# NathanBWaters/playaid_core

Measured on AMD Instinct MI355X. Metric: 1080p frames/sec end-to-end, higher is better.
Workload: dtype f32; 1 GPU; configs[1]: 64 x 1080x1920 BGR frames per GPU per clip; parallelism=single GPU, lanes=2, ingest=raw BGR frames resident in HBM

## Files before the change

### playaid_core_amd/csrc/engine_plan.h

```cpp
#pragma once
#include "gemm_tile.h"

#include <algorithm>
#include <cstddef>
#include <cstdlib>

namespace pa {

constexpr int WINO_F4_MIN_CROPS = 64;

struct EngineKnobs {
    int patch = 1;
    int bf16_patch = 1;
    int bf16_t256 = 1;
    int s2_pgemm = 2;
    int stem_igemm = 0;
    int stem_pool = 1;
    int pool_overlap = 1;
    int ds_side = 0;
    int stem_int = 1;
    int wino = 1;
    int wino_min_hw = 4;
    int wino_ds = 1;
    int wino_f4 = 1;
    int wino_f4_min = WINO_F4_MIN_CROPS;
    int bf16_ds_fuse = 1;
    int f32_ds_fuse = 1;
    bool profile_layers = false;
    int force_tile = -1;
    int force_splitk = 0;
    int fc_splitk = 0;
    int head_splitk = 0;
    int interleave = 0;
};

inline int env_int(const char* name, int unset) {
    const char* v = getenv(name);
    return v ? atoi(v) : unset;
}
inline int env_min1(const char* name) {
    const char* v = getenv(name);
    return v ? std::max(1, atoi(v)) : 0;
}

inline EngineKnobs engine_knobs() {
    static const EngineKnobs once = [] {
        EngineKnobs k;
        k.patch = env_int("PA_PATCH", k.patch);
        k.bf16_patch = env_int("PA_BF16_PATCH", k.bf16_patch);
        k.bf16_t256 = env_int("PA_BF16_T256", k.bf16_t256);
        k.s2_pgemm = env_int("PA_S2_PGEMM", k.s2_pgemm);
        k.stem_igemm = env_int("PA_STEM_IGEMM", k.stem_igemm);
        k.stem_pool = env_int("PA_STEM_POOL", k.stem_pool);
        k.pool_overlap = env_int("PA_POOL_OVERLAP", k.pool_overlap);
        k.ds_side = env_int("PA_DS_SIDE", k.ds_side);
        k.stem_int = env_int("PA_STEM_INT", k.stem_int);
        k.wino = env_int("PA_WINO", k.wino);
        k.wino_min_hw = env_int("PA_WINO_MIN_HW", k.wino_min_hw);
        k.wino_ds = env_int("PA_WINO_DS", k.wino_ds);
        k.wino_f4 = env_int("PA_WINO_F4", k.wino_f4);
        k.wino_f4_min = env_int("PA_WINO_F4_MIN", k.wino_f4_min);
        k.bf16_ds_fuse = env_int("PA_BF16_DS_FUSE", k.bf16_ds_fuse);
        k.f32_ds_fuse = env_int("PA_F32_DS_FUSE", k.f32_ds_fuse);
        return k;
    }();
    EngineKnobs k = once;
    const char* pl = getenv("PA_PROFILE_LAYERS");
    k.profile_layers = pl && pl[0] == '1';
    k.force_tile = env_int("PA_FORCE_TILE", -1);
    k.force_splitk = env_min1("PA_FORCE_SPLITK");
    k.fc_splitk = env_min1("PA_FC_SPLITK");
    k.head_splitk = env_min1("PA_HEAD_SPLITK");
    k.interleave = env_int("PA_INTERLEAVE", 0);
    return k;
}

enum ComputeDtype { DT_F32, DT_EMULATED_F32, DT_BF16 };

struct EngineForms {
    bool stem_fused;
    bool stem_int;
    bool opener_branch;
};
inline EngineForms engine_forms(const EngineKnobs& k, ComputeDtype dt) {
    EngineForms f;
    f.stem_fused = k.stem_pool && !k.stem_igemm;
    f.stem_int = dt != DT_BF16 && k.stem_int && f.stem_fused;
    f.opener_branch = dt == DT_BF16 ? k.bf16_ds_fuse != 0 : dt == DT_F32 && k.f32_ds_fuse && !k.ds_side && k.s2_pgemm;
    return f;
}

enum BranchPlace {
    BRANCH_NONE,
    BRANCH_SECOND_K,
// ... 209 lines not shown
```

### playaid_core_amd/csrc/pa_api.hip

```cpp
#include "../../include/playaid_hip.h"
#include "conv_rows.h"
#include "engine_table.h"
#include "synth_math.h"
#include "train_common.h"

#include <algorithm>
#include <cmath>
#include <cstdio>
#include <cstdlib>
#include <cstring>
#include <string>
#include <vector>

using namespace pa;

namespace {

static_assert(FEATURE_STRIDE == PA_FEATURE_STRIDE, "engine_table.h pads the fc to the cached feature rows' width");
constexpr int WINO_TICKETS = 4096;

struct ConvLayer : LayerDesc {
    std::string name;
    float* in = nullptr;
    float* out = nullptr;
// ... 246 lines not shown
            on = false;
            return;
        }
        (void)hipEventRecord(ent.start, s);
    }
    ~ProfScope() {
        if (!on) return;
        (void)hipEventRecord(ent.stop, s);
        e->prof_log.push_back(ent);
    }
};

float* buf_at(float* base, size_t elems, bool bf) { return reinterpret_cast<float*>(reinterpret_cast<char*>(base) + elems * (bf ? 2 : 4)); }

bool branch_on_side(const pa_engine* e, hipStream_t s) { return e->knobs.ds_side && !e->profiling && !e->bf16 && e->side && s != e->side; }

int run_branch_gemm(pa_engine* e, const ConvLayer& L, const BranchPlan& b, int crop0, int ncrops, size_t slab_off, hipStream_t s, const char* prof_name) {
    const int hw = L.branch.hw, c = L.branch.c, out_w = L.out_hw + 2 * L.out_pad;
    const size_t out_crop = (size_t)out_w * out_w * L.cout;
    GemmParams d = conv_row_params({ ncrops,  hw, hw, 1, c,
                                     c, L.cout, 1, L.branch.stride,
                                     L.out_pad, L.cout,  0, 0});
    d.act = buf_at(L.ds.src, (size_t)crop0 * (hw + 2) * (hw + 2) * c, e->bf16);
    d.wgt = L.ds.wgt;
    d.out = buf_at(L.ds.out, crop0 * out_crop, e->bf16);
    d.slab = e->slab + slab_off;
    ProfScope ps(e, s, prof_name, b.acct.flops, b.acct.bytes);
    if (e->bf16) HIPCHK(e, launch_igemm_bf16(d, b.tile, s));
    else if (b.psgemm) HIPCHK(e, launch_psgemm(d, L.ds.split_wgt, (size_t)ncrops * out_crop, 0, s));
    else HIPCHK(e, launch_igemm(d, b.tile, s));
    return PA_OK;
}

int run_conv(pa_engine* e, const ConvLayer& L, int crop0, int ncrops, size_t slab_off, hipStream_t s, const char* prof_name) {
    const size_t slab_avail = e->slab_floats > slab_off ? e->slab_floats - slab_off : 0;
    const ConvPlan P = plan_conv(e->knobs, e->dtype, L, ncrops, slab_avail, branch_on_side(e, s));
    const bool bf = e->bf16 && L.kh == 3;
    const int in_w = L.in_hw + 2 * L.in_pad;
    const int out_w = L.out_hw + 2 * L.out_pad;
    const size_t in_crop = (size_t)in_w * in_w * L.in_px_stride;
    const size_t out_crop = (size_t)out_w * out_w * L.cout;
    GemmParams p;
    memset(&p, 0, sizeof(p));
    p.act = buf_at(L.in, crop0 * in_crop, bf);
    p.wgt = L.wgt;
    p.bias = L.bias;
    p.residual = L.residual ? buf_at(L.residual, crop0 * out_crop, bf) : nullptr;
    p.out = buf_at(L.out, crop0 * out_crop, bf);
    p.slab = e->slab + slab_off;
    p.gather = nullptr;
    p.M = P.M;
    p.N = P.N;
    p.taps = L.taps;
    p.kw_taps = L.kw_taps;
    p.chunk = L.chunk;
    p.ktot = P.ktot;
    p.skip_w = L.kh == 7;
    p.howo = L.out_hw * L.out_hw;
    p.wo = L.out_hw;
    p.in_px_stride = L.in_px_stride;
    p.in_row_stride = in_w * L.in_px_stride;
    p.in_img_stride = (int)in_crop;
    p.stride = L.stride;
    p.off_y = L.off;
    p.off_x = L.off;
    p.out_px_stride = L.cout;
    p.out_row_stride = out_w * L.cout;
// ... 7 lines not shown
    }
    if (P.branch == BL_GEMM_BEFORE || P.branch == BL_STORED) {
        p.residual = buf_at(L.ds.out, crop0 * out_crop, bf);
    } else if (P.branch == BL_SECOND_K) {
        const int w2 = L.branch.hw + 2;
        p.act2 = buf_at(L.ds.src, (size_t)crop0 * w2 * w2 * L.branch.c, bf);
        p.k2_steps = L.branch.c / (bf ? 64 : 32);
        p.in2_px_stride = L.branch.c;
        p.in2_row_stride = w2 * L.branch.c;
        p.in2_img_stride = w2 * w2 * L.branch.c;
        p.stride2 = L.branch.stride;
        p.off2 = 1;
    }
    const ConvLayer* C2 = L.carries_of >= 0 ? &e->convs[L.carries_of] : nullptr;
    if (bf && P.branch == BL_ON_OPENER) {
        p.wgt2 = C2->ds.wgt;
        p.out2 = buf_at(C2->ds.out, crop0 * out_crop, bf);
    }
    bool branch_left = P.branch == BL_GEMM_BEHIND;
    {
        ProfScope ps(e, s, prof_name, P.acct.flops, P.acct.bytes, P.acct.flops_executed);
        hipError_t pe = hipErrorInvalidValue;
        if (P.form == CONV_PSGEMM) {
            pe = launch_psgemm(p, L.split_wgt, (size_t)ncrops * out_crop, 0, s);
        } else if (P.form == CONV_WINO && P.wino_f4) {
            Wino4Params q{};
            q.act = p.act; q.wgt = L.wino4_wgt; q.bias = p.bias; q.residual = p.residual; q.out = p.out;
            q.v = e->wino4_scratch + (slab_off ? e->wino4_region : 0);
            q.m = q.v + (size_t)36 * wino4_rows(ncrops) * L.cin;
            q.n_img = ncrops; q.cin = L.cin; q.cout = L.cout;
            q.in_px_stride = p.in_px_stride; q.in_row_stride = p.in_row_stride; q.in_img_stride = p.in_img_stride;
            q.out_px_stride = p.out_px_stride; q.out_row_stride = p.out_row_stride; q.out_img_stride = p.out_img_stride; q.out_pad = p.out_pad;
            q.relu = p.relu; q.res_after = p.res_after;
            pe = launch_wino4_conv3x3(q, s);
        } else if (P.form == CONV_WINO) {
            WinoParams q = wino_params(p, ncrops, L.out_hw, L.out_hw, L.cin, L.wino_wgt, L.wino_bn);
            if (e->wino_tickets && e->slab) {
                q.slab = e->slab + slab_off;
                q.slab_floats = e->slab_floats > slab_off ? std::min(e->slab_floats - slab_off, e->slab_floats / 2) : 0;
                q.tickets = reinterpret_cast<int32_t*>(e->wino_tickets) + (slab_off ? WINO_TICKETS : 0);
                q.tickets_cap = WINO_TICKETS;
            }
            pe = launch_wino3x3(q, s);
        } else if (bf) {
            if (P.form == CONV_BF16_PATCH) pe = launch_conv3x3_bf16_patch(p, s);
            if (pe == hipErrorInvalidValue) pe = launch_igemm_bf16(p, P.tile_256 ? TILE_256x128 : P.tile, s);
        } else {
            if (P.form == CONV_PATCH) pe = launch_conv3x3_patch(p, P.patch_bm, s);
            if (P.form == CONV_PGEMM && P.branch == BL_ON_OPENER) {
                p.wgt2 = C2->ds.wgt;
                p.out2 = buf_at(C2->ds.out, crop0 * out_crop, bf);
                pe = launch_pgemm(p, 64, s);
                branch_left = pe != hipSuccess;
                p.wgt2 = nullptr;
                p.out2 = nullptr;
            }
            if (P.form == CONV_PGEMM && pe == hipErrorInvalidValue) pe = launch_pgemm(p, P.pgemm_bm, s);
            if (pe == hipErrorInvalidValue) pe = launch_igemm(p, P.tile, s);
        }
        HIPCHK(e, pe);
    }
    if (branch_left) return run_branch_gemm(e, *C2, P.branch_gemm, crop0, ncrops, slab_off, s, e->knobs.profile_layers ? C2->name.c_str() : prof_name);
    return PA_OK;
}

int run_backbone_part(pa_engine* e, int crop0, int ncrops, const float* x_in, float* feats_out, size_t slab_off, hipStream_t s,
// ... 32 lines not shown
        memset(&sp, 0, sizeof(sp));
        const size_t es_in = x_form ? 2 : 4, es_out = e->bf16 ? 2 : 4;
        sp.x = reinterpret_cast<const char*>(x_in) + (size_t)crop0 * 134 * 134 * 4 * es_in;
        sp.wgt = x_form == 2 ? (const void*)e->stem_wgt_int : e->bf16 ? (const void*)e->stem_wgt_bf16 : (const void*)stem.wgt;
        sp.bias = stem.bias;
        sp.out = reinterpret_cast<char*>(e->p1) + (size_t)crop0 * 34 * 34 * 64 * es_out;
        sp.crops = ncrops;
        sp.in_bf16 = x_form;
        sp.out_bf16 = e->bf16 ? 1 : 0;
        const double px = (double)ncrops * 64 * 64;
        ProfScope ps(e, s, "stem_conv7x7_pool", 2.0 * px * 64 * 147,
                     (double)es_in * ((double)ncrops * 128 * 128 * 4 + 64.0 * 147 * (x_form == 2 ? 3 : 1)) + (double)es_out * ncrops * 32 * 32 * 64);
        HIPCHK(e, launch_stem_pool(sp, s));
    } else if (x_form == 2) {
        return fail(e, PA_ERR_INVALID_ARG, "integer pixels reached an unfused stem (PA_STEM_POOL=0 / PA_STEM_IGEMM=1 switch the integer stem off)");
    } else if (e->bf16) {
        return fail(e, PA_ERR_INVALID_ARG, "the bf16 path has no unfused stem (PA_STEM_POOL=0 / PA_STEM_IGEMM=1 are fp32 A/B knobs)");
    } else if (K.pool_overlap && !e->profiling && !K.interleave && e->side && s != e->side && ncrops >= 64) {
        const int half = (ncrops / 2 + 7) & ~7;
        if ((rc = stem_part(crop0, half, s))) return rc;
        HIPCHK(e, hipEventRecord(e->ev_fork, s));
        HIPCHK(e, hipStreamWaitEvent(e->side, e->ev_fork, 0));
        if ((rc = pool_part(crop0, half, e->side))) return rc;
        HIPCHK(e, hipEventRecord(e->ev_join, e->side));
        if ((rc = stem_part(crop0 + half, ncrops - half, s))) return rc;
        if ((rc = pool_part(crop0 + half, ncrops - half, s))) return rc;
        HIPCHK(e, hipStreamWaitEvent(s, e->ev_join, 0));
    } else {
        if ((rc = stem_part(crop0, ncrops, s))) return rc;
        if ((rc = pool_part(crop0, ncrops, s))) return rc;
    }
    if (stop <= 1) return PA_OK;
    const bool on_side = branch_on_side(e, s);
    for (size_t i = 1; i < e->convs.size(); ++i) {
        const ConvLayer& L = e->convs[i];
        const char* pn = K.profile_layers ? L.name.c_str() : (L.kh == 3 ? "igemm_conv3x3" : "igemm_conv1x1_ds");
        const bool side_next = on_side && i + 1 < e->convs.size() && e->convs[i + 1].branch.place == BRANCH_OWN_GEMM;
        if (side_next) {
            const ConvLayer& Nx = e->convs[i + 1];
            HIPCHK(e, hipEventRecord(e->ev_ds_fork, s));
            HIPCHK(e, hipStreamWaitEvent(e->side, e->ev_ds_fork, 0));
            if ((rc = run_branch_gemm(e, Nx, plan_branch(e->dtype, Nx, ncrops), crop0, ncrops, slab_off, e->side, "igemm_conv1x1_ds"))) return rc;
            HIPCHK(e, hipEventRecord(e->ev_ds_join, e->side));
        }
        if (on_side && L.branch.place == BRANCH_OWN_GEMM) HIPCHK(e, hipStreamWaitEvent(s, e->ev_ds_join, 0));
        if ((rc = run_conv(e, L, crop0, ncrops, slab_off, s, pn))) return rc;
        if (stop <= (int)i + 1) {
            if (side_next) HIPCHK(e, hipStreamWaitEvent(s, e->ev_ds_join, 0));
            return PA_OK;
        }
    }
    {
        ProfScope ps(e, s, "avgpool", 0.0, ncrops * ((e->bf16 ? 2.0 : 4.0) * 16.0 * 512 + 4.0 * 512));
        if (e->bf16)
            HIPCHK(e, launch_avgpool_bf16(reinterpret_cast<uint16_t*>(e->layer4_out) + (size_t)crop0 * 36 * 512,
                                          e->pooled + (size_t)crop0 * 512, ncrops, s));
        else
            HIPCHK(e, launch_avgpool(e->layer4_out + (size_t)crop0 * 36 * 512, e->pooled + (size_t)crop0 * 512, ncrops, s));
    }
    if (stop <= 18) return PA_OK;
    ConvLayer fc = e->fc;
    fc.out = feats_out;
    rc = run_conv(e, fc, crop0, ncrops, slab_off, s, "igemm_fc");
    return rc;
}

int run_backbone(pa_engine* e, int ncrops, const float* x_in, float* feats_out, hipStream_t s, int stop = PA_TRACE_STAGES) {
    if (!e->knobs.interleave || ncrops < 64 || !e->side) return run_backbone_part(e, 0, ncrops, x_in, feats_out, 0, s, stop);
    const int half = (ncrops / 2 + 7) & ~7;
    HIPCHK(e, hipEventRecord(e->ev_fork, s));
    HIPCHK(e, hipStreamWaitEvent(e->side, e->ev_fork, 0));
    int rc = run_backbone_part(e, 0, half, x_in, feats_out, 0, s, stop);
    if (rc) return rc;
    rc = run_backbone_part(e, half, ncrops - half, x_in, feats_out, e->slab_floats / 2, e->side, stop);
    if (rc) return rc;
    HIPCHK(e, hipEventRecord(e->ev_join, e->side));
    HIPCHK(e, hipStreamWaitEvent(s, e->ev_join, 0));
    return PA_OK;
}
// ... 1649 lines not shown
```

### playaid_core_amd/csrc/pa_kernels.h

```cpp
#pragma once
#include "gemm_tile.h"
#include <hip/hip_runtime.h>
#include <stdint.h>
#include "crop_math.h"

namespace pa {

__device__ __forceinline__ float silu_fast(float x) {
    return x * __builtin_amdgcn_rcpf(1.0f + __builtin_amdgcn_exp2f(x * -1.44269504088896341f));
}

struct GemmParams {
    const float* act;
    const float* wgt;
    const float* bias;
    const float* residual;
    float* out;
    float* slab;
    const int32_t* gather;
    int32_t M, N, ktot;
    int32_t taps, kw_taps, chunk;
    int32_t howo, wo;
    int32_t howo_shift, wo_shift;
    int32_t in_img_stride, in_row_stride, in_px_stride, stride, off_y, off_x;
// ... 82 lines not shown
    float* out;
    int32_t n_img, height, width, cin, cout;
    int32_t bn;
    int32_t in_px_stride, in_row_stride, in_img_stride;
    int32_t out_px_stride, out_row_stride, out_img_stride, out_pad;
    int32_t relu, res_after;
    int32_t n_sb, sb_per_row, sb_per_img, tiles_n;
    unsigned long long* clk;
    float* slab;
    size_t slab_floats;
    int32_t* tickets;
    int32_t tickets_cap, ksplit;
    int32_t tiles_m, xcd_gm, xcd_gn;
};
size_t wino_weight_floats(int cin, int cout);
int wino_pick_bn(int cout, long long n_sb, int cin_split = 0);
void wino_transform_weights(const float* w, int cin, int cout, int bn, float* ug);
hipError_t launch_wino3x3(const WinoParams& p, hipStream_t s);

struct Wino4Params {
    const float* act;
    const float* wgt;
    const float* bias;
    const float* residual;
    float* out;
    float* v;
    float* m;
    int32_t n_img, cin, cout;
    int32_t in_px_stride, in_row_stride, in_img_stride;
    int32_t out_px_stride, out_row_stride, out_img_stride, out_pad;
    int32_t relu, res_after;
    int32_t tile;
    int32_t rows;
};
size_t wino4_weight_floats(int cin, int cout);
int wino4_rows(int n_img);
void wino4_transform_weights(const float* w, int cin, int cout, float* u);
hipError_t launch_wino4_conv3x3(const Wino4Params& p, hipStream_t s);

#define PA_FUSED_LDS_BYTES 77824

#define PA_HOP_BLOCKS_MAX 48
#define PA_HOP_PIXELS 10
#define PA_HOP_WINDOW 64
#define PA_HOP_BLOCK_BYTES (6 * 1024 + 32 * 4 + 16)
#define PA_CROP_MFMA_H_DEFAULT 1

struct CropWindow {
    int64_t offset;
    int32_t pitch;
    int32_t rows;
    int64_t src_offset;
    int32_t src_pitch;
    int32_t row_bytes;
};
hipError_t launch_slice_upload(const uint8_t* frames_host, long long frames_bytes, const CropWindow* desc, uint8_t* windows, int ncrops,
                               hipStream_t s);

struct PreprocParams {
    const uint8_t* frames;
    const CropWindow* windows;
    const double* boxes;
    const int32_t* src_frame;
    int32_t n_src;
    int32_t n_frames, height, width, fighters, padding, swap_rb;
    CropPlan* plans;
// ... 229 lines not shown
```

### playaid_core_amd/csrc/pigemm.hip

```cpp
#include "pgemm_common.h"

#include <algorithm>
#include <type_traits>
#include <cstdio>
#include <cstdlib>
#include <vector>

namespace pa {


namespace {

typedef __attribute__((address_space(3))) float lds_f32;
typedef __attribute__((address_space(3))) f32x4 lds_f32x4;

template <int N> __device__ __forceinline__ void pg_wait_vm() { wait_vmcnt<(N > 63 ? 63 : N)>(); }

}

template <int BM, int BN, bool SILU, bool STAMP, bool UP, bool DS, bool GRP = false>
__device__ __forceinline__ void pgemm_body(const GemmParams& p) {
    static_assert(!DS || (!UP && !STAMP && !SILU), "the branch form is the ResNet openers': ReLU, no up-sampled copy");
    static_assert(!GRP || (!UP && !STAMP && !SILU && !DS), "the grouped form is a plain product");
    auto stamp = [&](int i) {
        if (STAMP) {
            const unsigned long long t = __builtin_amdgcn_s_memtime();
            if ((threadIdx.x & 63) == 0) p.clk[((size_t)blockIdx.x * 4 + (threadIdx.x >> 6)) * 64 + i] = t;
        }
    };
    stamp(0);
    constexpr int WM = BN == 64 ? 2 : 4;
    constexpr int MI = BM / WM / 32;
    constexpr int A_ROWS = BM / 32, B_ROWS = BN / 32;
    constexpr int NLD = A_ROWS + B_ROWS;
    constexpr int NST = MI * 4 * (UP ? 5 : (DS ? 2 : 1));
    constexpr int STAGE = (BM + BN + (DS ? BN : 0)) * 32;
    __shared__ __attribute__((aligned(16))) float lds[3 * STAGE];

    const TileRun run = tile_run(p);
    const int tile_n = run.tile_n, nt = run.nt;
    {
        const float *pa_ = p.act, *pw_ = p.wgt, *pb_ = p.bias;
        float* po_ = p.out;
        const int i0 = p.M, i1 = p.ktot, i2 = p.kw_taps, i3 = p.chunk, i4 = p.howo, i5 = p.wo, i6 = p.in_img_stride, i7 = p.in_row_stride,
                  i8 = p.in_px_stride, i9 = p.stride, i10 = p.off_y, i11 = p.off_x, i12 = p.out_img_stride, i13 = p.out_row_stride,
                  i14 = p.out_px_stride, i15 = p.out_pad, i16 = p.pg_ho, i17 = p.pg_nwx, i18 = p.pg_nwy;
        const unsigned u0 = p.pg_magic_howo, u1 = p.pg_magic_wo;
        asm volatile("" ::"s"(pa_), "s"(pw_), "s"(pb_), "s"(po_), "s"(i0), "s"(i1), "s"(i2), "s"(i3), "s"(i4), "s"(i5), "s"(i6), "s"(i7), "s"(i8), "s"(i9),
                     "s"(i10), "s"(i11), "s"(i12), "s"(i13), "s"(i14), "s"(i15), "s"(i16), "s"(i17), "s"(i18), "s"(u0), "s"(u1));
        if (DS) {
            const float* pw2_ = p.wgt2;
            float* po2_ = p.out2;
            asm volatile("" ::"s"(pw2_), "s"(po2_));
        }
        if (GRP) {
            const int g0 = p.grp_tiles, g1 = p.grp_wgt_bytes;
// ... 73 lines not shown
        const int tapoff = cur.tap_offset(p) * 4;
#pragma unroll
        for (int i = 0; i < A_ROWS; ++i) glds16(act_rs, a_off[i], tapoff, As_w + i * 1024);
        const int koff = ((cur.ky * p.kw_taps + cur.kx) * p.chunk + cur.kc) * 4 + (GRP ? w_grp : 0);
#pragma unroll
        for (int i = 0; i < B_ROWS; ++i) glds16(wgt_rs, b_off[i], koff, Bs_w + i * 1024);
        if (DS && cur.ky == 1 && cur.kx == 1) {
#pragma unroll
            for (int i = 0; i < B_ROWS; ++i) glds16(wgt2_rs, b2_off[i], cur.kc * 4, Bs_w + BN * 32 + i * 1024);
        }
        cur.advance(p, nk, run, rows_of);
    };

    unsigned a_k[4], b_k[4];
    {
        const int a_rd = (wm * (BM / WM) + lr) * 32, b_rd = BM * 32 + (wn * 32 + lr) * 32;
        const int swz = (lr >> 1) & 7;
        const unsigned base = (unsigned)(size_t)(lds_f32*)lds;
#pragma unroll
        for (int kk = 0; kk < 4; ++kk) {
            const int ch_ = ((kk * 2 + lh) ^ swz) * 4;
            a_k[kk] = base + (a_rd + ch_) * 4;
            b_k[kk] = base + (b_rd + ch_) * 4;
            asm volatile("" : "+v"(a_k[kk]), "+v"(b_k[kk]));
        }
    }

    issue(0);
    stamp(62);
    if (total > 1) issue(1);
    f32x16 biasv;
#pragma unroll
    for (int g = 0; g < 4; ++g) {
        const f32x4 b4 = p.bias ? *reinterpret_cast<const f32x4*>(p.bias + ch0 + 8 * g) : f32x4{0.f, 0.f, 0.f, 0.f};
        biasv[4 * g] = b4.x; biasv[4 * g + 1] = b4.y; biasv[4 * g + 2] = b4.z; biasv[4 * g + 3] = b4.w;
    }
    asm volatile("" : "+v"(biasv));
    stamp(1);

    f32x16 acc[MI];
    f32x16 acc2[MI];
    f32x16 accg[GRP ? 3 : 1][MI];
    auto kstep = [&](int sb, auto first_c, auto branch_c) {
        constexpr bool FIRST = decltype(first_c)::value;
        constexpr int BR = decltype(branch_c)::value;
        f32x16 zero16;
        if (BR == 1) {
#pragma unroll
            for (int e = 0; e < 16; ++e) zero16[e] = 0.f;
        }
        f32x4 b2f[2];
        unsigned ra[4], rb[4];
#pragma unroll
        for (int kk = 0; kk < 4; ++kk) {
            ra[kk] = a_k[kk] + sb;
            rb[kk] = b_k[kk] + sb;
            asm volatile("" : "+v"(ra[kk]), "+v"(rb[kk]));
        }
        f32x4 af[2][MI], bf[2];
#define PG_FRAGS(SET, KK)                                                                                    \
    {                                                                                                        \
        _Pragma("unroll") for (int mi = 0; mi < MI; ++mi)                                                    \
            af[SET][mi] = *(const lds_f32x4*)(size_t)(ra[KK] + mi * 4096);                                   \
        bf[SET] = *(const lds_f32x4*)(size_t)(rb[KK]);                                                       \
        if (BR) b2f[SET] = *(const lds_f32x4*)(size_t)(rb[KK] + BN * 128);                                    \
    }
        PG_FRAGS(0, 0);
#pragma unroll
        for (int kk = 0; kk < 4; ++kk) {
#pragma unroll
// ... 83 lines not shown
            }
            if (DS && live) {
                float* o2_px = p.out2 + o_off;
#pragma unroll
                for (int gq = 0; gq < 4; ++gq)
                    *reinterpret_cast<f32x4*>(o2_px + 8 * gq) = f32x4{acc2[mi][4 * gq], acc2[mi][4 * gq + 1], acc2[mi][4 * gq + 2], acc2[mi][4 * gq + 3]};
            }
            if (UP && live) {
                float* u_px = p.up_out + pixel_walk(geom, m_base, lr, p.up_img_stride, up_rs, up_ps, up_wrap_x, up_wrap_y, up_lane);
#pragma unroll
                for (int q4 = 0; q4 < 4; ++q4) {
                    float* u = u_px + (q4 >> 1) * p.up_row_stride + (q4 & 1) * p.up_px_stride;
#pragma unroll
                    for (int gq = 0; gq < 4; ++gq) *reinterpret_cast<f32x4*>(u + 8 * gq) = out4[gq];
                }
            }
        }
        if (t < 15) stamp(5 + 4 * t);
    }
    stamp(63);
}

template <int BM, int BN = 64, bool SILU = true, bool STAMP = false, bool UP = false>
__global__ __launch_bounds__(256, 2) void pgemm_kernel(const GemmParams p) {
    pgemm_body<BM, BN, SILU, STAMP, UP, false>(p);
}

__global__ __launch_bounds__(256, 2) void pgemm_branch_kernel(const GemmParams p) {
    pgemm_body<64, 64, false, false, false, true>(p);
}

template <int BM, int BN>
__global__ __launch_bounds__(256, 2) void pgemm_group_kernel(const GemmParams p) {
    pgemm_body<BM, BN, false, false, false, false, true>(p);
}

hipError_t launch_pgemm(const GemmParams& p_in, int bm, hipStream_t s) {
    GemmParams p = p_in;
    if (p.residual || p.N % 32 != 0 || (bm != 128 && bm != 64 && bm != 0) || persistent_plan(p) != hipSuccess) return hipErrorInvalidValue;
    const bool branch = p.wgt2 || p.out2;
    if (branch) {
        if (!p.wgt2 || !p.out2 || p.taps != 9 || p.kw_taps != 3 || p.stride != 2 || p.in_px_stride != p.chunk || p.splitk > 1 || p.N % 64 != 0 || p.relu == 2 || p.up_out ||
            ((reinterpret_cast<unsigned long long>(p.wgt2) | reinterpret_cast<unsigned long long>(p.out2)) & 15ull))
            return hipErrorInvalidValue;
        bm = 64;
    }
    const int bn = p.N % 64 == 0 ? 64 : 32;
    if (bn == 32) bm = 128;
    p.tiles_n = p.N / bn;
    if (p.tiles_n > 64) return hipErrorInvalidValue;
    auto plan = [&](int bm_, int* lm_out) {
        const int tm = (p.M + bm_ - 1) / bm_, share = (tm + 7) / 8;
        int lm = 64 / p.tiles_n;
        lm = lm < 1 ? 1 : (lm > share ? share : lm);
        *lm_out = lm;
        return (double)((share + lm - 1) / lm) * (bm_ == 128 ? 1.0 : 0.55) * (lm * p.tiles_n <= 32 ? 0.6 : 1.0);
    };
    int lm = 1;
    if (bm == 0) {
        int lm128, lm64;
        const double e128 = plan(128, &lm128), e64 = plan(64, &lm64);
        bm = e128 <= e64 ? 128 : 64;
        lm = bm == 128 ? lm128 : lm64;
    } else {
        (void)plan(bm, &lm);
    }
    p.tiles_m = (p.M + bm - 1) / bm;
// ... 45 lines not shown
hipError_t launch_pgemm_grouped(const float* a, const float* w, float* out, int groups, int rows, int K, int N, int tile, hipStream_t s) {
    auto mis = [](const void* q) { return (reinterpret_cast<unsigned long long>(q) & 15ull) != 0; };
    if (!a || !w || !out || mis(a) || mis(w) || mis(out) || groups < 1 || rows < 64 || rows % 64 || rows >= (1 << 16) || K < 32 || K % 32 || N < 64 || N % 64 ||
        tile < 0 || tile > 3)
        return hipErrorInvalidValue;
    if ((long long)groups * rows * K * 4 >= (1ll << 31) || (long long)groups * N * K * 4 >= (1ll << 31) || (long long)groups * rows * N >= (1ll << 31))
        return hipErrorInvalidValue;
    if (tile == 0) tile = 1;
    if (tile != 1 && rows % 128) tile = 1;
    const int bm = tile == 1 ? 64 : 128, bn = tile == 3 ? 32 : 64;
    GemmParams p;
    memset(&p, 0, sizeof(p));
    p.act = a; p.wgt = w; p.out = out;
    p.M = groups * rows; p.N = N; p.ktot = K;
    p.taps = 1; p.kw_taps = 1; p.chunk = K;
    p.howo = rows; p.wo = rows;
    p.in_px_stride = K; p.in_row_stride = rows * K; p.in_img_stride = rows * K; p.stride = 1;
    p.out_px_stride = N; p.out_row_stride = rows * N; p.out_img_stride = rows * N;
    p.splitk = 1;
    if (persistent_plan(p) != hipSuccess) return hipErrorInvalidValue;
    p.tiles_n = N / bn;
    p.tiles_m = p.M / bm;
    if (p.tiles_n > 64) return hipErrorInvalidValue;
    p.grp_tiles = rows / bm;
    p.grp_wgt_bytes = N * K * 4;
    p.grp_magic = (unsigned)std::min<unsigned long long>(((1ull << 32) + p.grp_tiles - 1) / p.grp_tiles, 0xffffffffull);
    const int share = (p.tiles_m + 7) / 8;
    int lm = 96 / p.tiles_n;
    static const int lm_force = getenv("PA_PGEMM_GROUP_LM") ? atoi(getenv("PA_PGEMM_GROUP_LM")) : 0;
    if (lm_force > 0) lm = lm_force;
    lm = lm < 1 ? 1 : (lm > share ? share : lm);
    p.pg_per = lm * p.tiles_n;
    const int grid = p.pg_per * 8;
    if (tile == 1) hipLaunchKernelGGL((pgemm_group_kernel<64, 64>), dim3(grid), dim3(256), 0, s, p);
    else if (tile == 2) hipLaunchKernelGGL((pgemm_group_kernel<128, 64>), dim3(grid), dim3(256), 0, s, p);
    else hipLaunchKernelGGL((pgemm_group_kernel<128, 32>), dim3(grid), dim3(256), 0, s, p);
    return hipGetLastError();
}

}
```

### playaid_core_amd/csrc/wino4.hip

```cpp
#include "tile_common.h"

#include <cstdlib>

namespace pa {

namespace {

__device__ __forceinline__ f32x4 w4_fma(float a, f32x4 x, f32x4 y) {
    return f32x4{__builtin_fmaf(a, x.x, y.x), __builtin_fmaf(a, x.y, y.y), __builtin_fmaf(a, x.z, y.z), __builtin_fmaf(a, x.w, y.w)};
}

__device__ __forceinline__ void w4_bt(f32x4 (&d)[6]) {
    const f32x4 t0 = w4_fma(4.f, d[0], w4_fma(-5.f, d[2], d[4]));
    const f32x4 t5 = w4_fma(4.f, d[1], w4_fma(-5.f, d[3], d[5]));
    const f32x4 a = w4_fma(-4.f, d[2], d[4]), b = w4_fma(-4.f, d[1], d[3]);
    const f32x4 c = d[4] - d[2], e = d[3] - d[1];
    d[0] = t0; d[1] = a + b; d[2] = a - b; d[3] = w4_fma(2.f, e, c); d[4] = w4_fma(-2.f, e, c); d[5] = t5;
}

__device__ __forceinline__ void w4_at(const f32x4 (&m)[6], f32x4 (&y)[4]) {
    const f32x4 s = m[1] + m[2], d = m[1] - m[2], u = m[3] + m[4], v = m[3] - m[4];
    y[0] = (m[0] + s) + u;
    y[1] = w4_fma(2.f, v, d);
    y[2] = w4_fma(4.f, u, s);
    y[3] = w4_fma(8.f, v, d) + m[5];
}

__global__ __launch_bounds__(64) void wino4_input_kernel(const Wino4Params p) {
    const int cq_n = p.cin >> 2;
    const int idx = blockIdx.x * 64 + threadIdx.x;
    const int row = idx / cq_n, c = (idx - row * cq_n) * 4;
    if (row >= p.rows) return;
    float* v = p.v + (size_t)row * p.cin + c;
    const size_t plane = (size_t)p.rows * p.cin;
    if (row >= p.n_img) {
#pragma unroll
        for (int q = 0; q < 36; ++q) *reinterpret_cast<f32x4*>(v + q * plane) = f32x4{0.f, 0.f, 0.f, 0.f};
        return;
    }
    const float* x = p.act + (size_t)row * p.in_img_stride + c;
    f32x4 d[6][6];
#pragma unroll
    for (int i = 0; i < 6; ++i)
#pragma unroll
        for (int j = 0; j < 6; ++j) d[i][j] = *reinterpret_cast<const f32x4*>(x + i * p.in_row_stride + j * p.in_px_stride);
#pragma unroll
    for (int j = 0; j < 6; ++j) {
        f32x4 l[6];
#pragma unroll
        for (int i = 0; i < 6; ++i) l[i] = d[i][j];
        w4_bt(l);
#pragma unroll
        for (int i = 0; i < 6; ++i) d[i][j] = l[i];
    }
#pragma unroll
    for (int i = 0; i < 6; ++i) {
        w4_bt(d[i]);
#pragma unroll
        for (int j = 0; j < 6; ++j) *reinterpret_cast<f32x4*>(v + (i * 6 + j) * plane) = d[i][j];
    }
}

__global__ __launch_bounds__(64) void wino4_output_kernel(const Wino4Params p) {
    const int cq_n = p.cout >> 2;
    const int idx = blockIdx.x * 64 + threadIdx.x;
    const int row = idx / cq_n, c = (idx - row * cq_n) * 4;
    if (row >= p.n_img) return;
    const float* m = p.m + (size_t)row * p.cout + c;
    const size_t plane = (size_t)p.rows * p.cout;
    f32x4 t[4][6];
#pragma unroll
    for (int j = 0; j < 6; ++j) {
        f32x4 l[6], y[4];
#pragma unroll
        for (int i = 0; i < 6; ++i) l[i] = *reinterpret_cast<const f32x4*>(m + (i * 6 + j) * plane);
        w4_at(l, y);
#pragma unroll
        for (int i = 0; i < 4; ++i) t[i][j] = y[i];
    }
    const f32x4 bias4 = p.bias ? *reinterpret_cast<const f32x4*>(p.bias + c) : f32x4{0.f, 0.f, 0.f, 0.f};
    const size_t o00 = (size_t)row * p.out_img_stride + (size_t)p.out_pad * (p.out_row_stride + p.out_px_stride) + c;
    f32x4 res4[4][4];
#pragma unroll
    for (int oy = 0; oy < 4; ++oy)
#pragma unroll
        for (int ox = 0; ox < 4; ++ox)
            res4[oy][ox] = p.residual ? *reinterpret_cast<const f32x4*>(p.residual + o00 + (size_t)oy * p.out_row_stride + ox * p.out_px_stride)
                                      : f32x4{0.f, 0.f, 0.f, 0.f};
#pragma unroll
    for (int oy = 0; oy < 4; ++oy) {
        f32x4 y[4];
        w4_at(t[oy], y);
#pragma unroll
        for (int ox = 0; ox < 4; ++ox)
            *reinterpret_cast<f32x4*>(p.out + o00 + (size_t)oy * p.out_row_stride + ox * p.out_px_stride) = epilogue4(y[ox], bias4, res4[oy][ox], p.relu, p.res_after);
    }
}

}

size_t wino4_weight_floats(int cin, int cout) { return (size_t)36 * cin * cout; }

int wino4_rows(int n_img) { return (n_img + 63) / 64 * 64; }

void wino4_transform_weights(const float* w, int cin, int cout, float* u) {
    static const double Gm[6][3] = {{1.0 / 4, 0, 0},          {-1.0 / 6, -1.0 / 6, -1.0 / 6}, {-1.0 / 6, 1.0 / 6, -1.0 / 6},
                                    {1.0 / 24, 1.0 / 12, 1.0 / 6}, {1.0 / 24, -1.0 / 12, 1.0 / 6},  {0, 0, 1}};
    const size_t plane = (size_t)cout * cin;
    for (int co = 0; co < cout; ++co)
        for (int ci = 0; ci < cin; ++ci) {
            double g[3][3], tmp[6][3];
            for (int ky = 0; ky < 3; ++ky)
                for (int kx = 0; kx < 3; ++kx) g[ky][kx] = (double)w[((size_t)co * 9 + ky * 3 + kx) * cin + ci];
            for (int i = 0; i < 6; ++i)
                for (int kx = 0; kx < 3; ++kx) tmp[i][kx] = Gm[i][0] * g[0][kx] + Gm[i][1] * g[1][kx] + Gm[i][2] * g[2][kx];
            for (int i = 0; i < 6; ++i)
                for (int j = 0; j < 6; ++j)
                    u[(size_t)(i * 6 + j) * plane + (size_t)co * cin + ci] = (float)(tmp[i][0] * Gm[j][0] + tmp[i][1] * Gm[j][1] + tmp[i][2] * Gm[j][2]);
        }
}

hipError_t launch_wino4_conv3x3(const Wino4Params& p_in, hipStream_t s) {
    Wino4Params p = p_in;
    if (!p.act || !p.wgt || !p.out || !p.v || !p.m || p.n_img < 1 || p.cin < 64 || p.cin % 64 || p.cout < 64 || p.cout % 64 || p.in_px_stride < p.cin ||
        p.out_px_stride < p.cout || p.out_pad < 0)
        return hipErrorInvalidValue;
    auto mis = [](const void* q) { return (reinterpret_cast<unsigned long long>(q) & 15ull) != 0; };
    if (p.in_px_stride % 4 || p.out_px_stride % 4 || p.in_row_stride % 4 || p.in_img_stride % 4 || p.out_row_stride % 4 || p.out_img_stride % 4 || mis(p.act) ||
        mis(p.wgt) || mis(p.out) || mis(p.v) || mis(p.m) || (p.bias && mis(p.bias)) || (p.residual && mis(p.residual)))
        return hipErrorInvalidValue;
    p.rows = wino4_rows(p.n_img);
    const long long in_threads = (long long)p.rows * (p.cin / 4), out_threads = (long long)p.n_img * (p.cout / 4);
    if (in_threads >= (1ll << 31) || out_threads >= (1ll << 31)) return hipErrorInvalidValue;
    hipLaunchKernelGGL(wino4_input_kernel, dim3((unsigned)((in_threads + 63) / 64)), dim3(64), 0, s, p);
    static const int tile_env = getenv("PA_WINO_F4_TILE") ? atoi(getenv("PA_WINO_F4_TILE")) : 0;
    const hipError_t e = launch_pgemm_grouped(p.v, p.wgt, p.m, 36, p.rows, p.cin, p.cout, p.tile ? p.tile : tile_env, s);
    if (e != hipSuccess) return e;
    hipLaunchKernelGGL(wino4_output_kernel, dim3((unsigned)((out_threads + 63) / 64)), dim3(64), 0, s, p);
    return hipGetLastError();
}

}

#include "../../include/playaid_hip.h"

extern "C" {

size_t pa_wino4_weight_floats(int32_t cin, int32_t cout) {
    if (cin < 64 || cin % 64 || cout < 64 || cout % 64) return 0;
    return pa::wino4_weight_floats(cin, cout);
}

int pa_wino4_transform_weights(const float* w_host, int32_t cin, int32_t cout, float* u_host) {
    if (!w_host || !u_host || cin < 64 || cin % 64 || cout < 64 || cout % 64) return PA_ERR_INVALID_ARG;
    pa::wino4_transform_weights(w_host, cin, cout, u_host);
    return PA_OK;
}

int pa_wino4_conv3x3(const float* x, const float* u, const float* bias, const float* residual, float* out, int32_t n, int32_t height, int32_t width,
                     int32_t cin, int32_t cout, int32_t in_px_stride, int32_t out_px_stride, int32_t out_pad, int32_t act, int32_t res_after,
                     float* scratch, size_t scratch_floats, void* stream) {
    if (!x || !u || !out || !scratch || n < 1 || height != 4 || width != 4 || out_pad < 0 || act < 0 || act > 2 || cin < 64 || cin % 64 || cout < 64 ||
        cout % 64 || (reinterpret_cast<unsigned long long>(scratch) & 15ull))
        return PA_ERR_INVALID_ARG;
    const size_t rows = (size_t)pa::wino4_rows(n);
    if (scratch_floats < 36 * rows * ((size_t)cin + cout)) return PA_ERR_INVALID_ARG;
    pa::Wino4Params p{};
    p.act = x; p.wgt = u; p.bias = bias; p.residual = residual; p.out = out;
    p.v = scratch;
    p.m = scratch + 36 * rows * cin;
    p.n_img = n; p.cin = cin; p.cout = cout;
// ... 15 lines not shown
```

Baseline: 75100 frames/s.

## Chain Winograd F4 layers by fusing next input transform into output kernel

New measurement: 74810 frames/s. Within noise of the previous version (-0.4%).

```diff
diff --git a/playaid_core_amd/csrc/engine_plan.h b/playaid_core_amd/csrc/engine_plan.h
--- a/playaid_core_amd/csrc/engine_plan.h
+++ b/playaid_core_amd/csrc/engine_plan.h
@@ -24,6 +24,7 @@
     int wino_ds = 1;
     int wino_f4 = 1;
     int wino_f4_min = WINO_F4_MIN_CROPS;
+    int wino_f4_chain = 1;
     int bf16_ds_fuse = 1;
     int f32_ds_fuse = 1;
     bool profile_layers = false;
@@ -60,6 +61,7 @@
         k.wino_ds = env_int("PA_WINO_DS", k.wino_ds);
         k.wino_f4 = env_int("PA_WINO_F4", k.wino_f4);
         k.wino_f4_min = env_int("PA_WINO_F4_MIN", k.wino_f4_min);
+        k.wino_f4_chain = env_int("PA_WINO_F4_CHAIN", k.wino_f4_chain);
         k.bf16_ds_fuse = env_int("PA_BF16_DS_FUSE", k.bf16_ds_fuse);
         k.f32_ds_fuse = env_int("PA_F32_DS_FUSE", k.f32_ds_fuse);
         return k;
diff --git a/playaid_core_amd/csrc/pa_api.hip b/playaid_core_amd/csrc/pa_api.hip
--- a/playaid_core_amd/csrc/pa_api.hip
+++ b/playaid_core_amd/csrc/pa_api.hip
@@ -302,7 +302,10 @@
     return PA_OK;
 }
 
-int run_conv(pa_engine* e, const ConvLayer& L, int crop0, int ncrops, size_t slab_off, hipStream_t s, const char* prof_name) {
+struct Wino4Chain {
+    bool v_ready = false, write_next = false;
+};
+int run_conv(pa_engine* e, const ConvLayer& L, int crop0, int ncrops, size_t slab_off, hipStream_t s, const char* prof_name, Wino4Chain chain = {}) {
     const size_t slab_avail = e->slab_floats > slab_off ? e->slab_floats - slab_off : 0;
     const ConvPlan P = plan_conv(e->knobs, e->dtype, L, ncrops, slab_avail, branch_on_side(e, s));
     const bool bf = e->bf16 && L.kh == 3;
@@ -376,6 +379,8 @@
             q.in_px_stride = p.in_px_stride; q.in_row_stride = p.in_row_stride; q.in_img_stride = p.in_img_stride;
             q.out_px_stride = p.out_px_stride; q.out_row_stride = p.out_row_stride; q.out_img_stride = p.out_img_stride; q.out_pad = p.out_pad;
             q.relu = p.relu; q.res_after = p.res_after;
+            q.v_ready = chain.v_ready;
+            q.v_next = chain.write_next ? q.v : nullptr;
             pe = launch_wino4_conv3x3(q, s);
         } else if (P.form == CONV_WINO) {
             WinoParams q = wino_params(p, ncrops, L.out_hw, L.out_hw, L.cin, L.wino_wgt, L.wino_bn);
@@ -474,8 +479,20 @@
     }
     if (stop <= 1) return PA_OK;
     const bool on_side = branch_on_side(e, s);
+    auto runs_f4 = [&](const ConvLayer& C) {
+        const ConvPlan P = plan_conv(K, e->dtype, C, ncrops, e->slab_floats > slab_off ? e->slab_floats - slab_off : 0, on_side);
+        return P.form == CONV_WINO && P.wino_f4;
+    };
+    bool v_ready = false;
     for (size_t i = 1; i < e->convs.size(); ++i) {
         const ConvLayer& L = e->convs[i];
+        Wino4Chain chain;
+        chain.v_ready = v_ready;
+        if (K.wino_f4_chain && i + 1 < e->convs.size()) {
+            const ConvLayer& Nx = e->convs[i + 1];
+            chain.write_next = Nx.in == L.out && Nx.cin == L.cout && L.cout <= L.cin && L.out_pad == 1 && Nx.in_pad == 1 && runs_f4(L) && runs_f4(Nx);
+        }
+        v_ready = chain.write_next;
         const char* pn = K.profile_layers ? L.name.c_str() : (L.kh == 3 ? "igemm_conv3x3" : "igemm_conv1x1_ds");
         const bool side_next = on_side && i + 1 < e->convs.size() && e->convs[i + 1].branch.place == BRANCH_OWN_GEMM;
         if (side_next) {
@@ -486,7 +503,7 @@
             HIPCHK(e, hipEventRecord(e->ev_ds_join, e->side));
         }
         if (on_side && L.branch.place == BRANCH_OWN_GEMM) HIPCHK(e, hipStreamWaitEvent(s, e->ev_ds_join, 0));
-        if ((rc = run_conv(e, L, crop0, ncrops, slab_off, s, pn))) return rc;
+        if ((rc = run_conv(e, L, crop0, ncrops, slab_off, s, pn, chain))) return rc;
         if (stop <= (int)i + 1) {
             if (side_next) HIPCHK(e, hipStreamWaitEvent(s, e->ev_ds_join, 0));
             return PA_OK;
diff --git a/playaid_core_amd/csrc/pa_kernels.h b/playaid_core_amd/csrc/pa_kernels.h
--- a/playaid_core_amd/csrc/pa_kernels.h
+++ b/playaid_core_amd/csrc/pa_kernels.h
@@ -138,6 +138,8 @@
     int32_t relu, res_after;
     int32_t tile;
     int32_t rows;
+    float* v_next;
+    int32_t v_ready;
 };
 size_t wino4_weight_floats(int cin, int cout);
 int wino4_rows(int n_img);
diff --git a/playaid_core_amd/csrc/pigemm.hip b/playaid_core_amd/csrc/pigemm.hip
--- a/playaid_core_amd/csrc/pigemm.hip
+++ b/playaid_core_amd/csrc/pigemm.hip
@@ -18,10 +18,11 @@
 
 }
 
-template <int BM, int BN, bool SILU, bool STAMP, bool UP, bool DS, bool GRP = false>
+template <int BM, int BN, bool SILU, bool STAMP, bool UP, bool DS, bool GRP = false, bool GRP_Z = false>
 __device__ __forceinline__ void pgemm_body(const GemmParams& p) {
     static_assert(!DS || (!UP && !STAMP && !SILU), "the branch form is the ResNet openers': ReLU, no up-sampled copy");
     static_assert(!GRP || (!UP && !STAMP && !SILU && !DS), "the grouped form is a plain product");
+    static_assert(!GRP_Z || GRP, "only the grouped form is known to have no bias");
     auto stamp = [&](int i) {
         if (STAMP) {
             const unsigned long long t = __builtin_amdgcn_s_memtime();
@@ -161,10 +162,10 @@
     f32x16 biasv;
 #pragma unroll
     for (int g = 0; g < 4; ++g) {
-        const f32x4 b4 = p.bias ? *reinterpret_cast<const f32x4*>(p.bias + ch0 + 8 * g) : f32x4{0.f, 0.f, 0.f, 0.f};
+        const f32x4 b4 = !GRP_Z && p.bias ? *reinterpret_cast<const f32x4*>(p.bias + ch0 + 8 * g) : f32x4{0.f, 0.f, 0.f, 0.f};
         biasv[4 * g] = b4.x; biasv[4 * g + 1] = b4.y; biasv[4 * g + 2] = b4.z; biasv[4 * g + 3] = b4.w;
     }
-    asm volatile("" : "+v"(biasv));
+    if (!GRP_Z) asm volatile("" : "+v"(biasv));
     stamp(1);
 
     f32x16 acc[MI];
@@ -314,7 +315,10 @@
 
 template <int BM, int BN>
 __global__ __launch_bounds__(256, 2) void pgemm_group_kernel(const GemmParams p) {
-    pgemm_body<BM, BN, false, false, false, false, true>(p);
+    pgemm_body<BM, BN, false, false, false, false, true, true>(p);
+}
+__global__ __launch_bounds__(256, 2) void pgemm_group_biasv_kernel(const GemmParams p) {
+    pgemm_body<64, 64, false, false, false, false, true, false>(p);
 }
 
 hipError_t launch_pgemm(const GemmParams& p_in, int bm, hipStream_t s) {
@@ -426,7 +430,9 @@
     lm = lm < 1 ? 1 : (lm > share ? share : lm);
     p.pg_per = lm * p.tiles_n;
     const int grid = p.pg_per * 8;
-    if (tile == 1) hipLaunchKernelGGL((pgemm_group_kernel<64, 64>), dim3(grid), dim3(256), 0, s, p);
+    static const bool biasv = getenv("PA_PGEMM_GROUP_BIASV") && atoi(getenv("PA_PGEMM_GROUP_BIASV")) != 0;
+    if (tile == 1 && biasv) hipLaunchKernelGGL(pgemm_group_biasv_kernel, dim3(grid), dim3(256), 0, s, p);
+    else if (tile == 1) hipLaunchKernelGGL((pgemm_group_kernel<64, 64>), dim3(grid), dim3(256), 0, s, p);
     else if (tile == 2) hipLaunchKernelGGL((pgemm_group_kernel<128, 64>), dim3(grid), dim3(256), 0, s, p);
     else hipLaunchKernelGGL((pgemm_group_kernel<128, 32>), dim3(grid), dim3(256), 0, s, p);
     return hipGetLastError();
diff --git a/playaid_core_amd/csrc/wino4.hip b/playaid_core_amd/csrc/wino4.hip
--- a/playaid_core_amd/csrc/wino4.hip
+++ b/playaid_core_amd/csrc/wino4.hip
@@ -1,52 +1,49 @@
 #include "tile_common.h"
 
+#include <algorithm>
 #include <cstdlib>
 
 namespace pa {
 
 namespace {
 
-__device__ __forceinline__ f32x4 w4_fma(float a, f32x4 x, f32x4 y) {
-    return f32x4{__builtin_fmaf(a, x.x, y.x), __builtin_fmaf(a, x.y, y.y), __builtin_fmaf(a, x.z, y.z), __builtin_fmaf(a, x.w, y.w)};
-}
-
-__device__ __forceinline__ void w4_bt(f32x4 (&d)[6]) {
-    const f32x4 t0 = w4_fma(4.f, d[0], w4_fma(-5.f, d[2], d[4]));
-    const f32x4 t5 = w4_fma(4.f, d[1], w4_fma(-5.f, d[3], d[5]));
-    const f32x4 a = w4_fma(-4.f, d[2], d[4]), b = w4_fma(-4.f, d[1], d[3]);
-    const f32x4 c = d[4] - d[2], e = d[3] - d[1];
+typedef f32x2 V;
+__device__ __forceinline__ V w4_fma(float a, V x, V y) { return V{__builtin_fmaf(a, x.x, y.x), __builtin_fmaf(a, x.y, y.y)}; }
+__device__ __forceinline__ V w4_zero() { return V{0.f, 0.f}; }
+
+__device__ __forceinline__ V w4_epilogue(V v, V bias, V res, int relu, int res_after) {
+    const f32x4 r = epilogue4(f32x4{v.x, v.y, 0.f, 0.f}, f32x4{bias.x, bias.y, 0.f, 0.f}, f32x4{res.x, res.y, 0.f, 0.f}, relu, res_after);
+    return V{r.x, r.y};
+}
+
+__device__ __forceinline__ void w4_bt(V (&d)[6]) {
+    const V t0 = w4_fma(4.f, d[0], w4_fma(-5.f, d[2], d[4]));
+    const V t5 = w4_fma(4.f, d[1], w4_fma(-5.f, d[3], d[5]));
+    const V a = w4_fma(-4.f, d[2], d[4]), b = w4_fma(-4.f, d[1], d[3]);
+    const V c = d[4] - d[2], e = d[3] - d[1];
     d[0] = t0; d[1] = a + b; d[2] = a - b; d[3] = w4_fma(2.f, e, c); d[4] = w4_fma(-2.f, e, c); d[5] = t5;
 }
 
-__device__ __forceinline__ void w4_at(const f32x4 (&m)[6], f32x4 (&y)[4]) {
-    const f32x4 s = m[1] + m[2], d = m[1] - m[2], u = m[3] + m[4], v = m[3] - m[4];
+__device__ __forceinline__ void w4_at(const V (&m)[6], V (&y)[4]) {
+    const V s = m[1] + m[2], d = m[1] - m[2], u = m[3] + m[4], v = m[3] - m[4];
     y[0] = (m[0] + s) + u;
     y[1] = w4_fma(2.f, v, d);
     y[2] = w4_fma(4.f, u, s);
     y[3] = w4_fma(8.f, v, d) + m[5];
 }
 
-__global__ __launch_bounds__(64) void wino4_input_kernel(const Wino4Params p) {
-    const int cq_n = p.cin >> 2;
-    const int idx = blockIdx.x * 64 + threadIdx.x;
-    const int row = idx / cq_n, c = (idx - row * cq_n) * 4;
-    if (row >= p.rows) return;
-    float* v = p.v + (size_t)row * p.cin + c;
-    const size_t plane = (size_t)p.rows * p.cin;
-    if (row >= p.n_img) {
-#pragma unroll
-        for (int q = 0; q < 36; ++q) *reinterpret_cast<f32x4*>(v + q * plane) = f32x4{0.f, 0.f, 0.f, 0.f};
-        return;
-    }
-    const float* x = p.act + (size_t)row * p.in_img_stride + c;
-    f32x4 d[6][6];
-#pragma unroll
-    for (int i = 0; i < 6; ++i)
-#pragma unroll
-        for (int j = 0; j < 6; ++j) d[i][j] = *reinterpret_cast<const f32x4*>(x + i * p.in_row_stride + j * p.in_px_stride);
+typedef unsigned w4_u32x2 __attribute__((ext_vector_type(2)));
+__device__ __forceinline__ void w4_ld(V& v, __amdgpu_buffer_rsrc_t rs, unsigned voff, unsigned soff) {
+    v = __builtin_bit_cast(V, __builtin_amdgcn_raw_buffer_load_b64(rs, voff, soff, 0));
+}
+__device__ __forceinline__ void w4_st(V v, __amdgpu_buffer_rsrc_t rs, unsigned voff, unsigned soff) {
+    __builtin_amdgcn_raw_buffer_store_b64(__builtin_bit_cast(w4_u32x2, v), rs, voff, soff, 0);
+}
+
+__device__ __forceinline__ void w4_input_transform(V (&d)[6][6], __amdgpu_buffer_rsrc_t v_rs, unsigned off, unsigned plane) {
 #pragma unroll
     for (int j = 0; j < 6; ++j) {
-        f32x4 l[6];
+        V l[6];
 #pragma unroll
         for (int i = 0; i < 6; ++i) l[i] = d[i][j];
         w4_bt(l);
@@ -57,43 +54,90 @@
     for (int i = 0; i < 6; ++i) {
         w4_bt(d[i]);
 #pragma unroll
-        for (int j = 0; j < 6; ++j) *reinterpret_cast<f32x4*>(v + (i * 6 + j) * plane) = d[i][j];
-    }
-}
-
+        for (int j = 0; j < 6; ++j) w4_st(d[i][j], v_rs, off, (i * 6 + j) * plane);
+    }
+}
+
+__device__ __forceinline__ void w4_zero_rows(__amdgpu_buffer_rsrc_t v_rs, unsigned off, unsigned plane) {
+#pragma unroll
+    for (int q = 0; q < 36; ++q) w4_st(w4_zero(), v_rs, off, q * plane);
+}
+
+__global__ __launch_bounds__(64) void wino4_input_kernel(const Wino4Params p) {
+    constexpr int C = 2;
+    const int cq_n = p.cin / C;
+    const int idx = blockIdx.x * 64 + threadIdx.x;
+    const int row = idx / cq_n, c = (idx - row * cq_n) * C;
+    if (row >= p.rows) return;
+    const __amdgpu_buffer_rsrc_t x_rs = glds_rsrc(p.act), v_rs = glds_rsrc(p.v);
+    const unsigned v_off = ((unsigned)row * p.cin + c) * 4u, plane = (unsigned)p.rows * p.cin * 4u;
+    if (row >= p.n_img) {
+        w4_zero_rows(v_rs, v_off, plane);
+        return;
+    }
+    const unsigned x_off = ((unsigned)row * p.in_img_stride + c) * 4u;
+    V d[6][6];
+#pragma unroll
+    for (int i = 0; i < 6; ++i)
+#pragma unroll
+        for (int j = 0; j < 6; ++j) w4_ld(d[i][j], x_rs, x_off, (unsigned)(i * p.in_row_stride + j * p.in_px_stride) * 4u);
+    w4_input_transform(d, v_rs, v_off, plane);
+}
+
+template <bool CHAIN>
 __global__ __launch_bounds__(64) void wino4_output_kernel(const Wino4Params p) {
-    const int cq_n = p.cout >> 2;
+    constexpr int C = 2;
+    const int cq_n = p.cout / C;
     const int idx = blockIdx.x * 64 + threadIdx.x;
-    const int row = idx / cq_n, c = (idx - row * cq_n) * 4;
-    if (row >= p.n_img) return;
-    const float* m = p.m + (size_t)row * p.cout + c;
-    const size_t plane = (size_t)p.rows * p.cout;
-    f32x4 t[4][6];
+    const int row = idx / cq_n, c = (idx - row * cq_n) * C;
+    const unsigned m_off = ((unsigned)row * p.cout + c) * 4u, plane = (unsigned)p.rows * p.cout * 4u;
+    const __amdgpu_buffer_rsrc_t vn_rs = glds_rsrc(CHAIN ? p.v_next : p.m);
+    if (row >= p.n_img) {
+        if (CHAIN && row < p.rows) w4_zero_rows(vn_rs, m_off, plane);
+        return;
+    }
+    const __amdgpu_buffer_rsrc_t m_rs = glds_rsrc(p.m), out_rs = glds_rsrc(p.out), res_rs = glds_rsrc(p.residual ? p.residual : p.out);
+    V t[4][6];
 #pragma unroll
     for (int j = 0; j < 6; ++j) {
-        f32x4 l[6], y[4];
-#pragma unroll
-        for (int i = 0; i < 6; ++i) l[i] = *reinterpret_cast<const f32x4*>(m + (i * 6 + j) * plane);
+        V l[6], y[4];
+#pragma unroll
+        for (int i = 0; i < 6; ++i) w4_ld(l[i], m_rs, m_off, (i * 6 + j) * plane);
         w4_at(l, y);
 #pragma unroll
         for (int i = 0; i < 4; ++i) t[i][j] = y[i];
     }
-    const f32x4 bias4 = p.bias ? *reinterpret_cast<const f32x4*>(p.bias + c) : f32x4{0.f, 0.f, 0.f, 0.f};
-    const size_t o00 = (size_t)row * p.out_img_stride + (size_t)p.out_pad * (p.out_row_stride + p.out_px_stride) + c;
-    f32x4 res4[4][4];
+#pragma unroll
+    for (int i = 0; i < 4; ++i)
+#pragma unroll
+        for (int j = 0; j < 6; ++j) asm volatile("" : "+v"(t[i][j]) : : "memory");
+    const V bias = p.bias ? *reinterpret_cast<const V*>(p.bias + c) : w4_zero();
+    const unsigned o_off = ((unsigned)row * p.out_img_stride + c) * 4u;
+    const unsigned o00 = (unsigned)(p.out_pad * (p.out_row_stride + p.out_px_stride)) * 4u;
+    V res[4][4];
 #pragma unroll
     for (int oy = 0; oy < 4; ++oy)
 #pragma unroll
-        for (int ox = 0; ox < 4; ++ox)
-            res4[oy][ox] = p.residual ? *reinterpret_cast<const f32x4*>(p.residual + o00 + (size_t)oy * p.out_row_stride + ox * p.out_px_stride)
-                                      : f32x4{0.f, 0.f, 0.f, 0.f};
+        for (int ox = 0; ox < 4; ++ox) {
+            res[oy][ox] = w4_zero();
+            if (p.residual) w4_ld(res[oy][ox], res_rs, o_off, o00 + (unsigned)(oy * p.out_row_stride + ox * p.out_px_stride) * 4u);
+        }
+    V d[6][6];
 #pragma unroll
     for (int oy = 0; oy < 4; ++oy) {
-        f32x4 y[4];
+        V y[4];
         w4_at(t[oy], y);
 #pragma unroll
-        for (int ox = 0; ox < 4; ++ox)
-            *reinterpret_cast<f32x4*>(p.out + o00 + (size_t)oy * p.out_row_stride + ox * p.out_px_stride) = epilogue4(y[ox], bias4, res4[oy][ox], p.relu, p.res_after);
+        for (int ox = 0; ox < 4; ++ox) {
+            const V z = w4_epilogue(y[ox], bias, res[oy][ox], p.relu, p.res_after);
+            w4_st(z, out_rs, o_off, o00 + (unsigned)(oy * p.out_row_stride + ox * p.out_px_stride) * 4u);
+            if (CHAIN) d[oy + 1][ox + 1] = z;
+        }
+    }
+    if (CHAIN) {
+#pragma unroll
+        for (int i = 0; i < 6; ++i) d[0][i] = d[5][i] = d[i][0] = d[i][5] = w4_zero();
+        w4_input_transform(d, vn_rs, m_off, plane);
     }
 }
 
@@ -130,13 +174,25 @@
         mis(p.wgt) || mis(p.out) || mis(p.v) || mis(p.m) || (p.bias && mis(p.bias)) || (p.residual && mis(p.residual)))
         return hipErrorInvalidValue;
     p.rows = wino4_rows(p.n_img);
-    const long long in_threads = (long long)p.rows * (p.cin / 4), out_threads = (long long)p.n_img * (p.cout / 4);
+    {
+        const long long lim = 1ll << 31, ch = std::max(p.cin, p.cout);
+        if (36ll * p.rows * ch * 4 >= lim || (p.n_img + 1ll) * std::max(p.in_img_stride, p.out_img_stride) * 4 >= lim || p.in_row_stride < 0 || p.in_img_stride < 0 ||
+            p.out_row_stride < 0 || p.out_img_stride < 0)
+            return hipErrorInvalidValue;
+    }
+    if (p.v_next) {
+        const size_t span = (size_t)36 * p.rows * p.cout;
+        if (mis(p.v_next) || p.out_pad != 1 || (p.v_next < p.m + span && p.m < p.v_next + span)) return hipErrorInvalidValue;
+    }
+    const long long in_threads = (long long)p.rows * (p.cin / 2), out_threads = (long long)(p.v_next ? p.rows : p.n_img) * (p.cout / 2);
     if (in_threads >= (1ll << 31) || out_threads >= (1ll << 31)) return hipErrorInvalidValue;
-    hipLaunchKernelGGL(wino4_input_kernel, dim3((unsigned)((in_threads + 63) / 64)), dim3(64), 0, s, p);
+    const dim3 in_grid((unsigned)((in_threads + 63) / 64)), out_grid((unsigned)((out_threads + 63) / 64));
+    if (!p.v_ready) hipLaunchKernelGGL(wino4_input_kernel, in_grid, dim3(64), 0, s, p);
     static const int tile_env = getenv("PA_WINO_F4_TILE") ? atoi(getenv("PA_WINO_F4_TILE")) : 0;
     const hipError_t e = launch_pgemm_grouped(p.v, p.wgt, p.m, 36, p.rows, p.cin, p.cout, p.tile ? p.tile : tile_env, s);
     if (e != hipSuccess) return e;
-    hipLaunchKernelGGL(wino4_output_kernel, dim3((unsigned)((out_threads + 63) / 64)), dim3(64), 0, s, p);
+    if (p.v_next) hipLaunchKernelGGL(wino4_output_kernel<true>, out_grid, dim3(64), 0, s, p);
+    else hipLaunchKernelGGL(wino4_output_kernel<false>, out_grid, dim3(64), 0, s, p);
     return hipGetLastError();
 }
 
```
